# yewzijian/RegTR

Measured on AMD Instinct MI355X. Metric: point-cloud pairs/sec (3DMatch ~20k pts), higher is better.
Workload: dtype f32 (f16-pair split, 22-bit operands)

## Files before the change

### include/regtr_hip.h

```cpp
#ifndef REGTR_HIP_H
#define REGTR_HIP_H

#include <stddef.h>

#ifdef __cplusplus
extern "C" {
#endif

#define REGTR_OK 0
#define REGTR_ERR_LAUNCH (-1)
#define REGTR_ERR_ARG (-2)
#define REGTR_ERR_WORKSPACE (-3)

#define REGTR_ABI_VERSION 11
int regtr_abi_version(void);

#define REGTR_STATUS_F16_RANGE 1
#define REGTR_STATUS_NONFINITE_POSE 2


size_t regtr_grid_subsample_ws_bytes(int n_cap, int n_clouds);

int regtr_grid_subsample(const float* xyz, const int* seg_off, int n_clouds, int n_cap, float dl, float* out_xyz,
                         int* out_seg_off, void* ws, size_t ws_bytes, void* stream);

size_t regtr_grid_subsample_ordered_ws_bytes(int n_cap, int n_clouds, int row_order);
int regtr_grid_subsample_ordered(const float* xyz, const int* seg_off, int n_clouds, int n_cap, float dl, int row_order, int key_mode,
                                 int out_cap, float* out_xyz, int* out_seg_off, void* ws, size_t ws_bytes, void* stream);

size_t regtr_cellgrid_ws_bytes(int ns_cap, int n_clouds);

int regtr_cellgrid_build(const float* s_xyz, const int* s_seg_off, int n_clouds, int ns_cap, float radius, void* ws,
                         size_t ws_bytes, void* stream);

int regtr_radius_query(const float* q_xyz, const int* q_seg_off, int nq_cap, const int* s_seg_off, int ns_cap,
                       int n_clouds, float radius, int K, int order, const void* grid_ws, size_t ws_bytes, int* out_idx,
                       int* out_count, int* out_max_count, void* stream);

int regtr_radius_query_self(const int* s_seg_off, int ns_cap, int n_clouds, float radius, int K, int order, const void* grid_ws,
                            size_t ws_bytes, int* out_idx, int* out_count, int* out_max_count, void* stream);


int regtr_nearest_in_radius(const float* q_xyz, const int* q_seg_off, int nq_cap, const int* s_seg_off, int ns_cap,
                            int n_clouds, double radius, float grid_radius, const void* grid_ws, size_t ws_bytes, int* out_idx,
                            void* stream);

int regtr_overlap_avgpool(const float* ov, int ns, const int* nbr, int ld_nbr, int nq, int H, float* out, void* stream);



int regtr_rowsum_positive(const float* x, int n, int C, const float* stats, const int* seg_off, int n_seg, float slope,
                          float* flag, void* stream);

int regtr_kpconv_gather_computes_flag(int Cin, int H);

int regtr_kpconv_gather(const float* q_xyz, int nq, const float* s_xyz, int ns, const int* nbr, int H, const float* x,
                        int Cin, const float* flag, const float* s_xyzf, const float* kernel_points, int KP, float extent,
                        const float* x_stats, const int* q_seg_off, int n_seg, float slope, float* wf, int ld_wf, float* num,
                        void* stream);

int regtr_maxpool_gather(const float* x, int ns, int C, const int* nbr, int ld_nbr, int nq, int H, float* out, void* stream);

size_t regtr_instnorm_ws_bytes(int n_clouds, int max_len, int C);
int regtr_instnorm_stats(const float* x, const int* seg_off, int n_clouds, int max_len, int C, float eps, float* stats,
                         void* ws, size_t ws_bytes, void* stream);
int regtr_instnorm_apply(const float* x, const int* seg_off, int n_clouds, int max_len, int C, const float* stats,
                         const float* residual, const float* res_stats, int act, float slope, float* y, const float* row_xyz,
                         float* row_positive, void* stream);


size_t regtr_gemm_f32_ws_bytes(int M, int N, int K);
int regtr_gemm_f32(const float* A, int lda, const float* B, int ldb, float* C, int ldc, int M, int N, int K,
                   const float* bias, const float* row_div, const float* residual, int ldr, int act,
                   const float* a_stats, const int* a_seg_off, int n_seg, float a_slope, void* ws, size_t ws_bytes,
                   void* stream);

int regtr_gemm_x3_supported(int M, int N, int K);
int regtr_gemm_x3_preferred(int M, int N, int K);
size_t regtr_gemm_split_weights_bytes(int N, int K);
int regtr_gemm_split_weights(const float* W, int ld, int N, int K, int transposed, void* planes, void* stream);
int regtr_gemm_x3_f16_supported(int M, int N, int K, int with_stats);
size_t regtr_gemm_split_weights_f16_bytes(int N, int K);
int regtr_gemm_split_weights_f16(const float* W, int ld, int N, int K, int transposed, void* planes, void* stream);
size_t regtr_gemm_x3_ws_bytes(int M, int N, int K);
int regtr_gemm_x3(const float* A, int lda, const void* planes, float* C, int ldc, int M, int N, int K,
                  const float* bias, const float* row_div, const float* residual, int ldr, int act,
                  const float* a_stats, const int* a_seg_off, int n_seg, float a_slope, void* ws, size_t ws_bytes,
                  double* stat_partial, const int* stat_seg_off, int n_stat_seg, int n_planes, const void* tile_info, int* status,
                  void* stream);
int regtr_tile_segments(const int* seg_off, int n_seg, int M, int rows, void* out, void* stream);
int regtr_gemm_x3_tile_rows(int M, int N, int K);
int regtr_gemm_stream_supported(int M, int N, int K);
int regtr_gemm_stream_tile_rows(void);
int regtr_gemm_stream(const float* A, int lda, const void* planes, float* C, int ldc, int M, int N, int K,
                      const float* a_stats, float a_slope, const int* seg_off, int n_seg, const void* tile_info,
                      double* stat_partial, void* stream);
int regtr_block_tail_supported(int M, int N, int K1, int K2);
size_t regtr_block_tail_ws_bytes(int n_clouds, int max_len, int N, int K1, int K2);
int regtr_block_tail(const float* A1, int lda1, const float* a1_stats, float a1_slope, const float* row_div1, const float* A2, int lda2,
                     const float* W1, const float* W2, const int* seg_off, int n_clouds, int max_len, const void* tile_info,
                     int M, int N, int K1, int K2, float eps, float slope, float* Y, int ldy, void* ws, size_t ws_bytes,
                     float* out_stats, void* stream);

int regtr_gemm_x3_stat_tile_rows(int M, int N, int K);
int regtr_instnorm_finalize_tiles(const double* partial, const int* seg_off, int n_clouds, int C, int tile_rows, float eps,
                                  float* stats, void* stream);

int regtr_add_f32(const float* a, const float* b, size_t n, float* out, void* stream);

int regtr_layernorm(const float* x, int n, int D, const float* gamma, const float* beta, float eps, const float* add,
                    float* y, float* y_plain, void* stream);

int regtr_posemb_sine(const float* xyz, int n, int npf, int d_model, float scale, const float* dim_t, float* pe,
                      void* stream);

int regtr_posemb_mlp(const float* xyz, int n, const float* const* w_kn, const float* const* bias, int d_model, float* pe, float* acts,
                     void* stream);


int regtr_mha_fwd(const float* q, int ldq, const float* k, int ldk, const float* v, int ldv, float* out, int ldo,
                  const int* seg_off, const int* kv_of, int n_clouds, int max_len, int n_heads, int head_dim, float scale,
                  int precision, int* status, void* stream);

int regtr_cross_encoder_per_layer_params(void);
int regtr_cross_encoder_supported(int n_tok, int d_model, int d_ff, int n_heads);
size_t regtr_cross_encoder_ws_bytes(int n_tok, int d_model, int d_ff);
int regtr_cross_encoder_fwd(const float* x, int n_tok, int d_model, int d_ff, int n_heads, int n_layers,
                            const void* const* layer_params, const float* layer_eps, const float* final_gamma,
                            const float* final_beta, float final_eps, int return_intermediate, const float* pe,
                            const int* seg_off, const int* kv_self, const int* kv_cross, int n_clouds, int max_len,
                            int gemm_planes, int attn_precision, void* ws, size_t ws_bytes, float* outs, int* status, void* stream);

typedef struct {
    const float* kn;
    const void* planes;
    const void* planes16;
    int N, K;
} regtr_weight_t;
typedef struct {
    int kind;
    int strided;
    int layer;
    int n_kp;
    float extent;
    const float* kernel_points;
    regtr_weight_t unary1;
    regtr_weight_t conv;
    regtr_weight_t unary2;
    regtr_weight_t shortcut;
} regtr_encoder_block_t;
typedef struct {
    const float* points;
    int n;
    const int* conv_idx;
    const int* pool_idx;
    int K;
    int pool_width;
    const int* seg_off;
    int max_len;
} regtr_encoder_level_t;
int regtr_encoder_supported(const regtr_encoder_block_t* blocks, int n_blocks, const regtr_encoder_level_t* levels, int n_levels,
                            int n_clouds, int first, int last);
size_t regtr_encoder_ws_bytes(const regtr_encoder_block_t* blocks, int n_blocks, const regtr_encoder_level_t* levels, int n_levels,
                              int n_clouds, int first, int last, int f16_pair);
int regtr_encoder_fwd(const regtr_encoder_block_t* blocks, int n_blocks, const regtr_encoder_level_t* levels, int n_levels, int n_clouds,
                      int first, int last, const float* x_in, float* out, int f16_pair, float slope, float eps, void* ws, size_t ws_bytes,
                      int* status, void* stream);

int regtr_attn_xyz(const float* q, const float* k, const float* xyz, float* out, const int* seg_off, const int* kv_of,
                   int n_clouds, int n_total, int n_layers, int max_len, int head_dim, float scale, void* stream);

int regtr_weighted_procrustes(const float* kp, const float* corr, const float* logit, const int* seg_off, int n_pairs,
                              int n_total, int n_layers, float* pose, int* status, void* stream);

int regtr_weighted_procrustes_bwd(const float* kp, const float* corr, const float* logit, const int* seg_off, int n_pairs, int n_total,
                                  int n_layers, const float* d_pose, float* d_corr, float* d_logit, float* d_kp, float* d_weight,
                                  void* stream);


// ... 215 lines not shown
```

### regtr_amd/_lib.py

```python
import ctypes
import os
import threading

import torch

from . import context

_HERE = os.path.dirname(os.path.abspath(__file__))
LIB_PATH = os.path.join(_HERE, 'libregtr_hip.so')
if os.environ.get('REGTR_DEV', '') == '1' and os.environ.get('REGTR_VARIANT'):
    LIB_PATH = os.path.join(_HERE, f"libregtr_hip.{os.environ['REGTR_VARIANT']}.so")

_c = ctypes
_P = _c.c_void_p
_I = _c.c_int
_F = _c.c_float
_Z = _c.c_size_t
_U64 = _c.c_uint64
_U32 = _c.c_uint32
_P5 = _c.POINTER(_c.c_void_p * 5)

class Weight(_c.Structure):
    _fields_ = [('kn', _P), ('planes', _P), ('planes16', _P), ('N', _I), ('K', _I)]


class EncoderBlock(_c.Structure):
    _fields_ = [('kind', _I), ('strided', _I), ('layer', _I), ('n_kp', _I), ('extent', _F), ('kernel_points', _P),
                ('unary1', Weight), ('conv', Weight), ('unary2', Weight), ('shortcut', Weight)]


class EncoderLevel(_c.Structure):
    _fields_ = [('points', _P), ('n', _I), ('conv_idx', _P), ('pool_idx', _P), ('K', _I), ('pool_width', _I), ('seg_off', _P), ('max_len', _I)]


ABI_VERSION = 11

PARITY_SIGNATURES = {
    'regtr_parity_abi_version': (_I, []),
    'regtr_kdtree_ws_bytes': (_Z, [_I, _I]),
    'regtr_kdtree_query_scratch_bytes': (_Z, [_I]),
    'regtr_kdtree_build': (_I, [_P, _P, _I, _I, _P, _Z, _P]),
    'regtr_kdtree_radius_query': (_I, [_P, _P, _I, _P, _P, _I, _I, _F, _I, _I, _P, _Z, _P, _Z, _P, _P, _P, _P, _P]),
}

SIGNATURES = {
    'regtr_abi_version': (_I, []),
    'regtr_grid_subsample_ws_bytes': (_Z, [_I, _I]),
    'regtr_grid_subsample': (_I, [_P, _P, _I, _I, _F, _P, _P, _P, _Z, _P]),
    'regtr_grid_subsample_ordered_ws_bytes': (_Z, [_I, _I, _I]),
    'regtr_grid_subsample_ordered': (_I, [_P, _P, _I, _I, _F, _I, _I, _I, _P, _P, _P, _Z, _P]),
    'regtr_cellgrid_ws_bytes': (_Z, [_I, _I]),
    'regtr_cellgrid_build': (_I, [_P, _P, _I, _I, _F, _P, _Z, _P]),
    'regtr_radius_query': (_I, [_P, _P, _I, _P, _I, _I, _F, _I, _I, _P, _Z, _P, _P, _P, _P]),
    'regtr_radius_query_self': (_I, [_P, _I, _I, _F, _I, _I, _P, _Z, _P, _P, _P, _P]),
    'regtr_nearest_in_radius': (_I, [_P, _P, _I, _P, _I, _I, _c.c_double, _F, _P, _Z, _P, _P]),
    'regtr_overlap_avgpool': (_I, [_P, _I, _P, _I, _I, _I, _P, _P]),
    'regtr_rowsum_positive': (_I, [_P, _I, _I, _P, _P, _I, _F, _P, _P]),
    'regtr_kpconv_gather_computes_flag': (_I, [_I, _I]),
    'regtr_kpconv_gather': (_I, [_P, _I, _P, _I, _P, _I, _P, _I, _P, _P, _P, _I, _F, _P, _P, _I, _F, _P, _I, _P, _P]),
    'regtr_maxpool_gather': (_I, [_P, _I, _I, _P, _I, _I, _I, _P, _P]),
    'regtr_instnorm_ws_bytes': (_Z, [_I, _I, _I]),
    'regtr_instnorm_stats': (_I, [_P, _P, _I, _I, _I, _F, _P, _P, _Z, _P]),
    'regtr_instnorm_apply': (_I, [_P, _P, _I, _I, _I, _P, _P, _P, _I, _F, _P, _P, _P, _P]),
    'regtr_gemm_f32_ws_bytes': (_Z, [_I, _I, _I]),
    'regtr_gemm_f32': (_I, [_P, _I, _P, _I, _P, _I, _I, _I, _I, _P, _P, _P, _I, _I, _P, _P, _I, _F, _P, _Z, _P]),
    'regtr_gemm_x3_supported': (_I, [_I, _I, _I]),
    'regtr_gemm_x3_preferred': (_I, [_I, _I, _I]),
    'regtr_gemm_split_weights_bytes': (_Z, [_I, _I]),
    'regtr_gemm_split_weights': (_I, [_P, _I, _I, _I, _I, _P, _P]),
    'regtr_gemm_x3_f16_supported': (_I, [_I, _I, _I, _I]),
    'regtr_gemm_split_weights_f16_bytes': (_Z, [_I, _I]),
    'regtr_gemm_split_weights_f16': (_I, [_P, _I, _I, _I, _I, _P, _P]),
    'regtr_gemm_x3_ws_bytes': (_Z, [_I, _I, _I]),
    'regtr_gemm_x3': (_I, [_P, _I, _P, _P, _I, _I, _I, _I, _P, _P, _P, _I, _I, _P, _P, _I, _F, _P, _Z, _P, _P, _I, _I, _P, _P, _P]),
    'regtr_tile_segments': (_I, [_P, _I, _I, _I, _P, _P]),
    'regtr_gemm_x3_tile_rows': (_I, [_I, _I, _I]),
    'regtr_gemm_stream_supported': (_I, [_I, _I, _I]),
    'regtr_gemm_stream_tile_rows': (_I, []),
    'regtr_block_tail_supported': (_I, [_I, _I, _I, _I]),
    'regtr_block_tail_ws_bytes': (_Z, [_I, _I, _I, _I, _I]),
    'regtr_block_tail': (_I, [_P, _I, _P, _F, _P, _P, _I, _P, _P, _P, _I, _I, _P, _I, _I, _I, _I, _F, _F, _P, _I, _P, _Z, _P, _P]),
    'regtr_gemm_stream': (_I, [_P, _I, _P, _P, _I, _I, _I, _I, _P, _F, _P, _I, _P, _P, _P]),
    'regtr_gemm_x3_stat_tile_rows': (_I, [_I, _I, _I]),
    'regtr_instnorm_finalize_tiles': (_I, [_P, _P, _I, _I, _I, _F, _P, _P]),
    'regtr_add_f32': (_I, [_P, _P, _Z, _P, _P]),
    'regtr_layernorm': (_I, [_P, _I, _I, _P, _P, _F, _P, _P, _P, _P]),
    'regtr_posemb_sine': (_I, [_P, _I, _I, _I, _F, _P, _P, _P]),
    'regtr_posemb_mlp': (_I, [_P, _I, _P5, _P5, _I, _P, _P, _P]),
    'regtr_mha_fwd': (_I, [_P, _I, _P, _I, _P, _I, _P, _I, _P, _P, _I, _I, _I, _I, _F, _I, _P, _P]),
    'regtr_cross_encoder_per_layer_params': (_I, []),
    'regtr_cross_encoder_supported': (_I, [_I, _I, _I, _I]),
    'regtr_cross_encoder_ws_bytes': (_Z, [_I, _I, _I]),
    'regtr_cross_encoder_fwd': (_I, [_P, _I, _I, _I, _I, _I, _P, _P, _P, _P, _F, _I, _P, _P, _P, _P, _I, _I, _I, _I, _P, _Z, _P, _P, _P]),
    'regtr_encoder_supported': (_I, [_P, _I, _P, _I, _I, _I, _I]),
    'regtr_encoder_ws_bytes': (_Z, [_P, _I, _P, _I, _I, _I, _I, _I]),
    'regtr_encoder_fwd': (_I, [_P, _I, _P, _I, _I, _I, _I, _P, _P, _I, _F, _F, _P, _Z, _P, _P]),
    'regtr_attn_xyz': (_I, [_P, _P, _P, _P, _P, _P, _I, _I, _I, _I, _I, _F, _P]),
    'regtr_weighted_procrustes': (_I, [_P, _P, _P, _P, _I, _I, _I, _P, _P, _P]),
    'regtr_weighted_procrustes_bwd': (_I, [_P, _P, _P, _P, _I, _I, _I, _P, _P, _P, _P, _P, _P]),
    'regtr_infonce_ws_bytes': (_Z, [_I, _I]),
    'regtr_infonce': (_I, [_P, _I, _P, _I, _P, _P, _P, _P, _I, _I, _I, _I, _I, _F, _F, _P, _P, _P, _P, _P, _Z, _P]),
    'regtr_loss_terms': (_I, [_P, _P, _P, _P, _P, _I, _I, _P, _I, _P, _P]),
    'regtr_se3_transform': (_I, [_P, _P, _I, _I, _P, _I, _P, _P]),
    'regtr_infonce_rows': (_I, [_P, _I, _P, _I, _P, _P, _P, _P, _I, _I, _I, _I, _I, _F, _F, _P, _P, _P, _P, _P, _P, _P, _Z, _P]),
    'regtr_infonce_bwd': (_I, [_P, _I, _P, _I, _P, _P, _P, _P, _I, _I, _I, _I, _I, _I, _F, _P, _P, _P, _P, _P, _P, _F, _P, _I, _P, _I,
                               _P]),
    'regtr_circle_rows': (_I, [_P, _I, _P, _I, _P, _P, _P, _P, _I, _I, _I, _I, _I, _I, _F, _F, _F, _F, _F, _F, _F, _P, _P, _P, _P, _P, _P,
                               _P]),
    'regtr_circle_bwd': (_I, [_P, _I, _P, _I, _P, _P, _P, _P, _I, _I, _I, _I, _I, _I, _F, _F, _F, _F, _F, _F, _F, _P, _P, _P, _P, _P, _P,
                              _P, _F, _P, _I, _P, _I, _P]),
    'regtr_gemm_tn_ws_bytes': (_Z, [_I, _I, _I]),
    'regtr_gemm_tn': (_I, [_P, _I, _P, _I, _I, _I, _I, _I, _P, _I, _P, _Z, _P]),
    'regtr_corr_l1_bwd': (_I, [_P, _P, _P, _P, _I, _I, _P, _I, _P, _P, _P, _P]),
    'regtr_mha_bwd_ws_bytes': (_Z, [_I, _I]),
    'regtr_mha_bwd': (_I, [_P, _I, _P, _I, _P, _I, _P, _I, _P, _I, _P, _I, _P, _I, _P, _P, _I, _I, _I, _I, _I, _F, _P, _Z, _P]),
    'regtr_layernorm_bwd_ws_bytes': (_Z, [_I, _I]),
    'regtr_layernorm_bwd': (_I, [_P, _I, _I, _P, _F, _P, _P, _P, _P, _P, _P, _Z, _P]),
    'regtr_bias_relu_bwd_ws_bytes': (_Z, [_I, _I]),
    'regtr_bias_relu_bwd': (_I, [_P, _I, _P, _I, _P, _I, _P, _I, _I, _P, _Z, _P]),
    'regtr_nbr_transpose_ws_bytes': (_Z, [_I, _I, _I]),
    'regtr_nbr_transpose': (_I, [_P, _I, _I, _I, _P, _P, _P, _Z, _P]),
    'regtr_kpconv_gather_bwd': (_I, [_P, _P, _I, _P, _I, _I, _I, _P, _I, _F, _P, _P, _P, _P]),
    'regtr_row_div': (_I, [_P, _I, _P, _I, _I, _P, _I, _P]),
    'regtr_gemm_tn_any_ws_bytes': (_Z, [_I, _I, _I]),
    'regtr_gemm_tn_any': (_I, [_P, _I, _P, _I, _I, _I, _I, _P, _I, _P, _Z, _P]),
    'regtr_instnorm_bwd_ws_bytes': (_Z, [_I, _I, _I]),
    'regtr_instnorm_bwd': (_I, [_P, _P, _I, _I, _I, _P, _P, _P, _I, _F, _P, _P, _P, _P, _Z, _P]),
    'regtr_maxpool_argmax': (_I, [_P, _I, _I, _P, _I, _I, _I, _P, _P]),
    'regtr_maxpool_fwd_argmax': (_I, [_P, _I, _I, _P, _I, _I, _I, _P, _P, _P]),
    'regtr_maxpool_gather_bwd': (_I, [_P, _P, _I, _I, _I, _P, _P, _I, _P, _P]),
    'regtr_head_tail_bwd_ws_bytes': (_Z, [_I, _I]),
    'regtr_head_tail_bwd': (_I, [_P, _P, _P, _P, _P, _P, _I, _I, _P, _P, _P, _P, _P, _P, _P, _P, _Z, _P]),
    'regtr_bce_logits_bwd': (_I, [_P, _P, _P, _I, _P, _P]),
    'regtr_cloud_centroids': (_I, [_P, _P, _I, _I, _P, _P]),
    'regtr_augment_draws': (_I, [_P, _I, _P, _I, _U64, _U32, _I, _F, _I, _P, _P, _P, _P]),
    'regtr_shuffle_keys': (_I, [_P, _I, _I, _U64, _U32, _P, _P]),
    'regtr_augment_gather': (_I, [_P, _P, _P, _I, _P, _P, _P, _I, _I, _P, _F, _U64, _U32, _P, _P, _P]),
    'regtr_modelnet_draws': (_I, [_I, _U64, _U32, _c.c_double, _c.c_double, _P, _P, _P, _P]),
    'regtr_crop_select_lds_points': (_I, []),
    'regtr_crop_select': (_I, [_P, _P, _I, _I, _I, _P, _P, _P, _P, _I, _P, _P, _P, _P, _P, _P]),
    'regtr_modelnet_keys': (_I, [_P, _I, _I, _I, _P, _U64, _U32, _P, _P]),
    'regtr_modelnet_gather': (_I, [_P, _P, _I, _I, _P, _I, _I, _P, _P, _P, _P, _F, _F, _U64, _U32, _P, _P, _P, _P]),
    'regtr_nearest_lds_points': (_I, []),
    'regtr_nearest': (_I, [_P, _P, _I, _P, _P, _I, _I, _I, _P, _P, _P, _P, _P]),
    'regtr_segment_mean': (_I, [_P, _P, _I, _I, _P, _P]),
    'regtr_pose_metrics': (_I, [_P, _P, _I, _I, _I, _P, _P, _P]),
    'regtr_optim_norm_slice': (_I, []),
    'regtr_optim_step_slice': (_I, []),
    'regtr_optim_chunk_tensors': (_I, []),
    'regtr_grad_sumsq': (_I, [_P, _I, _P, _c.c_longlong, _P]),
    'regtr_grad_norm_finish': (_I, [_P, _c.c_longlong, _F, _P, _P]),
    'regtr_adam_step': (_I, [_P, _I, _P, _I, _P]),
    'regtr_gather_segments': (_I, [_P, _P, _P, _I, _P, _I, _I, _P, _P, _I, _I, _I, _P, _P, _P, _P]),
    'regtr_grad_pack_slice': (_I, []),
    'regtr_grad_pack': (_I, [_P, _I, _P, _c.c_longlong, _F, _I, _P]),
    'regtr_grad_pack_guarded': (_I, [_P, _I, _P, _c.c_longlong, _F, _I, _P, _P, _P]),
    'regtr_optim_guarded_chunk_tensors': (_I, []),
    'regtr_grad_norm_finish_guarded': (_I, [_P, _c.c_longlong, _F, _P, _P, _P, _P]),
    'regtr_adam_step_guarded': (_I, [_P, _I, _P, _P, _c.c_longlong, _P, _P, _P, _I, _P]),
    'regtr_adam_bias_scalars': (_I, [_c.c_double, _c.c_double, _c.c_double, _P, _I, _P, _P]),
    'regtr_icp_chunk': (_I, []),
    'regtr_icp_ws_bytes': (_Z, [_I, _I]),
    'regtr_icp_step': (_I, [_P, _P, _I, _I, _P, _I, _I, _c.c_double, _F, _P, _Z, _P, _I, _I, _c.c_double, _c.c_double, _P, _P, _P, _P, _P,
                            _P, _Z, _P]),
}
# ... 122 lines not shown
```

### regtr_amd/csrc/gemm_stream.hip

```cpp
#include "common.h"
#include "mfma_operands.h"

namespace {

constexpr int SG_WAVES = 8;
constexpr int SG_ROWS = 32 * SG_WAVES;

struct SgArgs {
    const float* A; const uint16_t* Wt; float* C;
    const float2* a_stats;
    const int* seg_off;
    const int4* tile_info;
    double2* stat_partial;
    size_t plane;
    int M, N, Kp, lda, ldc, n_seg;
    float a_slope;
};

template <int KT> __device__ __forceinline__ unsigned sg_swz(unsigned n)
{
    constexpr int CPR = 2 * KT;
    return CPR == 4 ? ((n >> 2) & 3u) : (CPR == 8 ? ((n >> 1) & 7u) : (n & 15u));
}

// ... 70 lines not shown
                }
            }
            unsigned w[4][3];
#pragma unroll
            for (int e = 0; e < 4; e++) rg_split2(row_ok ? x[2 * e] : 0.f, row_ok ? x[2 * e + 1] : 0.f, w[e]);
#pragma unroll
            for (int p = 0; p < 3; p++) fa[ks][p] = __builtin_bit_cast(bf16x8, make_uint4(w[0][p], w[1][p], w[2][p], w[3][p]));
        }
    }
    SG_STAMP();
    unsigned f_off[KT];
#pragma unroll
    for (int ks = 0; ks < KT; ks++) f_off[ks] = (unsigned)l31 * ROWB + (((unsigned)(2 * ks + hi)) ^ sg_swz<KT>((unsigned)l31)) * 16u;

    floatx16 acc[NT];
#pragma unroll
    for (int j = 0; j < NT; j++)
#pragma unroll
        for (int r = 0; r < 16; r++) acc[j][r] = 0.f;
#pragma unroll
    for (int ks = 0; ks < KT; ks++)
#pragma unroll
        for (int j = 0; j < NT; j++) {
            bf16x8 fb[3];
#pragma unroll
            for (int p = 0; p < 3; p++)
                fb[p] = __builtin_bit_cast(bf16x8, *(const uint4*)(Ws + (size_t)(p * NB + 32 * j) * ROWB + f_off[ks]));
            acc[j] = __builtin_amdgcn_mfma_f32_32x32x16_bf16(fa[ks][2], fb[0], acc[j], 0, 0, 0);
            acc[j] = __builtin_amdgcn_mfma_f32_32x32x16_bf16(fa[ks][1], fb[1], acc[j], 0, 0, 0);
            acc[j] = __builtin_amdgcn_mfma_f32_32x32x16_bf16(fa[ks][0], fb[2], acc[j], 0, 0, 0);
            acc[j] = __builtin_amdgcn_mfma_f32_32x32x16_bf16(fa[ks][1], fb[0], acc[j], 0, 0, 0);
            acc[j] = __builtin_amdgcn_mfma_f32_32x32x16_bf16(fa[ks][0], fb[1], acc[j], 0, 0, 0);
            acc[j] = __builtin_amdgcn_mfma_f32_32x32x16_bf16(fa[ks][0], fb[0], acc[j], 0, 0, 0);
        }

    const int rbase = r0 + 4 * hi;
#ifdef SG_PROF
    { float z = 0.f; for (int j = 0; j < NT; j++) z += acc[j][0]; if (z == 1.2345e30f) pt[0] = 0; }
#endif
    SG_STAMP();
    if (g.stat_partial) {
    double2* red = (double2*)(Ws + (size_t)3 * NB * ROWB);
    for (int sg = s_lo; sg <= s_hi; sg++) {
        const int c_lo = sg == s_lo ? ti.z : g.seg_off[sg], c_hi = min(sg == s_lo ? ti.w : g.seg_off[sg + 1], g.M);
#pragma unroll
        for (int j = 0; j < NT; j++) {
            double s = 0.0, q = 0.0;
#pragma unroll
            for (int r = 0; r < 16; r++) {
                const int rw = rbase + (r & 3) + 8 * (r >> 2);
                if (rw >= c_lo && rw < c_hi) { const double v = (double)acc[j][r]; s += v; q += v * v; }
            }
            s += __shfl_xor(s, 32, RG_WAVE); q += __shfl_xor(q, 32, RG_WAVE);
            if (hi == 0) red[wave * NB + 32 * j + l31] = make_double2(s, q);
        }
        __syncthreads();
        if (t < NB) {
            double2 a = red[t];
#pragma unroll
            for (int w = 1; w < SG_WAVES; w++) { const double2 b = red[w * NB + t]; a.x += b.x; a.y += b.y; }
            g.stat_partial[(size_t)(row_tile + sg) * N + n0 + t] = a;
        }
        if (sg < s_hi) __syncthreads();
    }
    }
    SG_STAMP();
#pragma unroll
    for (int j = 0; j < NT; j++)
#pragma unroll
        for (int r = 0; r < 16; r++) {
            const int rw = rbase + (r & 3) + 8 * (r >> 2);
            if (rw < g.M) g.C[(size_t)rw * g.ldc + n0 + 32 * j + l31] = acc[j][r];
        }
#ifdef SG_PROF
    SG_STAMP();
    __builtin_amdgcn_s_waitcnt(0);
    SG_STAMP();
    if (lane == 0 && (row_tile == 700 || row_tile == 1500) && n0 == 0 && (wave == 0 || wave == 5))
        printf("gemm_strip KT %d NT %d row tile %d wave %d: loads+Wcopy %lld barrier %lld split %lld mfma %lld stats %lld store-issue %lld drain %lld total %lld\n", KT, NT, row_tile, wave,
               pt[1] - pt[0], pt[2] - pt[1], pt[3] - pt[2], pt[4] - pt[3], pt[5] - pt[4], pt[6] - pt[5], pt[7] - pt[6], pt[7] - pt[0]);
#endif
}

int sg_cols_per_wg(int N, int K)
{
    for (int nb = 128; nb >= 32; nb /= 2)
        if (nb <= N && N % nb == 0 && (size_t)nb * K * 6 + (size_t)SG_WAVES * nb * 16 <= 64 * 1024) return nb;
    return 0;
}

}

extern "C" {

int regtr_gemm_stream_supported(int M, int N, int K)
{
    return (M >= 0 && (K == 32 || K == 64 || K == 128) && N >= 32 && N <= 512 && N % 32 == 0 && sg_cols_per_wg(N, K) > 0) ? 1 : 0;
}

int regtr_gemm_stream_tile_rows(void) { return SG_ROWS; }

int regtr_gemm_stream(const float* A, int lda, const void* planes, float* C, int ldc, int M, int N, int K,
                      const float* a_stats, float a_slope, const int* seg_off, int n_seg, const void* tile_info,
                      double* stat_partial, void* stream)
{
    if (!A || !planes || !C || !regtr_gemm_stream_supported(M, N, K) || lda < K || ldc < N) return RG_ERR_ARG;
    if ((lda % 4) || ((uintptr_t)A % 16) || ((uintptr_t)planes % 16)) return RG_ERR_ARG;
    if (!seg_off || n_seg < 1 || !tile_info || ((uintptr_t)tile_info % 16)) return RG_ERR_ARG;
    if (a_stats && (K > 64 || ((uintptr_t)a_stats % 16))) return RG_ERR_ARG;
    if (stat_partial && ((uintptr_t)stat_partial % 16)) return RG_ERR_ARG;
    if (M == 0) return RG_OK;
    const RgPlaneDims pd = rg_plane_dims(N, K);
    SgArgs g{A, (const uint16_t*)planes, C, (const float2*)a_stats, seg_off, (const int4*)tile_info, (double2*)stat_partial,
             pd.elems(), M, N, pd.Kp, lda, ldc, n_seg, a_slope};
    const int NB = sg_cols_per_wg(N, K);
    hipStream_t st = (hipStream_t)stream;
    const size_t lds = (size_t)3 * NB * K * 2 + (size_t)SG_WAVES * NB * 16;
    const long long n_wg = (long long)rg_cdiv(rg_cdiv(M, SG_ROWS), 8) * 8 * (N / NB);
    if (n_wg > 0x7fffffffLL) return RG_ERR_ARG;
    const dim3 grid((unsigned)n_wg);
#define SG_L3(KT_, NT_) do { if (a_stats) k_gemm_strip<KT_, NT_, (KT_ <= 4)><<<grid, SG_WAVES * RG_WAVE, lds, st>>>(g); \
                             else k_gemm_strip<KT_, NT_, false><<<grid, SG_WAVES * RG_WAVE, lds, st>>>(g); } while (0)
#define SG_L2(KT_) do { if (NB == 32) SG_L3(KT_, 1); else if (NB == 64) SG_L3(KT_, 2); else SG_L3(KT_, 4); } while (0)
    if (K == 32) SG_L2(2);
    else if (K == 64) SG_L2(4);
    else SG_L2(8);
#undef SG_L2
#undef SG_L3
    RG_RETURN_IF_LAUNCH_FAILED();
    return RG_OK;
}

}
```

### regtr_amd/ops.py

```python
import functools
import math
import operator

import torch

from . import _lib, context
from ._lib import bptr, check, dptr, iptr, ptr, raw, stream


def _ws(nbytes, device):
    return torch.empty(int(nbytes), dtype=torch.uint8, device=device)


def _ws_as(numel, dtype, device):
    return _ws(int(numel) * dtype.itemsize, device).view(dtype)


F16_OPERAND_LIMIT = 65504.0 / 2


VOXEL_KEY_MODES = {'origin': 0, 'floor': 1, 'floor_rcp': 2}


def grid_subsample(xyz, seg_off, n_cap, dl, row_order=0, key_mode=0, out_cap=None):
# ... 181 lines not shown
    ldc = out.stride(0) if M > 1 else N
    n_seg = a_seg_off.numel() - 1 if a_stats is not None else 0
    x3_ok, x3_pref, nb, x3_R, x3_rows = _x3_plan(M, N, K) if sw is not None and sw.planes is not None else (False, False, 0, 0, 0)
    ctx = context.current()
    use_f16_pair = ctx.f16_pair and not ctx.force_x3
    if ctx.force_x3:
        planes = 3
    f16_range_log = ctx.f16_range_log
    if (x3_ok and lda % 4 == 0 and a.data_ptr() % 16 == 0 and not force_f32_gemm and (N >= 64 or a_stats is None)
            and (force_x3_gemm or x3_pref)):
        ws = _ws(nb, a.device) if nb else None
        R = x3_R if want_stats is not None else 0
        partial, s_off, n_clouds = None, None, 0
        if R:
            s_off = want_stats[0]
            n_clouds = s_off.numel() - 1
            partial = _ws_as(((M + R - 1) // R + n_clouds) * N * 2, torch.float64, a.device)
        seg_rows = s_off if R else a_seg_off
        ti = None
        if seg_rows is not None and (a_seg_off is None or s_off is None or a_seg_off is s_off):
            ti = tile_segments(seg_rows, M, x3_rows)
        pl, npl = sw.planes, int(planes)
        if use_f16_pair and npl >= 2 and sw.f16_ok and f16_pair_ok(M, N, K, R > 0 or a_stats is not None or ti is not None):
            pl, npl = sw.planes16, 4
            if f16_range_log is not None:
                f16_range_log.append((M, N, K, float(a.abs().max()) if M else 0.0, float(sw.kn.abs().max())))
        tm = _GemmTimer(ctx.gemm_records, M=M, N=N, K=K, route='split GEMM (f16 pair)' if npl == 4 else f'split GEMM (bf16 x{npl})',
                        terms={4: 3, 3: 6, 2: 3, 1: 1}[npl], w_bytes={4: 4, 3: 6, 2: 4, 1: 2}[npl], fold=a_stats is not None, stats=R > 0)
        check(L.regtr_gemm_x3(raw(a), lda, bptr(pl), raw(out), ldc, M, N, K, ptr(bias), ptr(row_div),
                              raw(residual), ldr, 1 if relu else 0,
                              ptr(a_stats), iptr(a_seg_off), n_seg, a_slope, bptr(ws), nb, dptr(partial), iptr(s_off), n_clouds,
                              npl, iptr(ti), ctx.status_ptr(), stream()), 'regtr_gemm_x3')
        tm.done()
        if R:
            stats = torch.empty((n_clouds, N, 2), dtype=torch.float32, device=a.device)
            check(L.regtr_instnorm_finalize_tiles(dptr(partial), iptr(s_off), n_clouds, N, R, eps, ptr(stats), stream()),
                  'regtr_instnorm_finalize_tiles')
            return out, stats
    else:
        nb = L.regtr_gemm_f32_ws_bytes(M, N, K)
        ws = _ws(nb, a.device) if nb else None
        tm = _GemmTimer(ctx.gemm_records, M=M, N=N, K=K, route='exact-f32 MFMA', terms=0, w_bytes=4, fold=a_stats is not None, stats=False)
        check(L.regtr_gemm_f32(raw(a), lda, ptr(b_kn), N, raw(out), ldc, M, N, K, ptr(bias), ptr(row_div),
                               raw(residual), ldr, 1 if relu else 0,
                               ptr(a_stats), iptr(a_seg_off), n_seg, a_slope, bptr(ws), nb, stream()), 'regtr_gemm_f32')
        tm.done()
    if want_stats is not None:
        return out, instnorm_stats(out, want_stats[0], want_stats[1], eps)
    return out


def tile_segments(seg_off, M, rows):
    cache = getattr(seg_off, '_regtr_tiles', None)
    if cache is None:
        cache = seg_off._regtr_tiles = {}
    key = (M, rows, seg_off.data_ptr(), seg_off._version)
    t = cache.get(key)
    if t is None:
        t = torch.empty(((M + rows - 1) // rows, 4), dtype=torch.int32, device=seg_off.device)
        check(_lib.lib().regtr_tile_segments(iptr(seg_off), seg_off.numel() - 1, M, rows, iptr(t), stream()), 'regtr_tile_segments')
        for k in [k for k in cache if k[2:] != key[2:]]:
            del cache[k]
        cache[key] = t
    return t


def stream_ok(M, N, K, a, a_stats=None):
    return bool(use_stream_gemm and not force_f32_gemm and not force_x3_gemm and M >= STREAM_MIN_ROWS and a.stride(1) == 1
                and a.stride(0) % 4 == 0 and a.data_ptr() % 16 == 0 and (a_stats is None or K <= 64)
                and _lib.lib().regtr_gemm_stream_supported(M, N, K))


def gemm_stream(a, sw, seg_off, a_stats=None, a_slope=0.1, want_stats=False, eps=1e-5):
    L = _lib.lib()
    M, K = a.shape
    N = sw.N
    n_clouds = seg_off.numel() - 1
    R = L.regtr_gemm_stream_tile_rows()
    ti = tile_segments(seg_off, M, R)
    partial = None
    if want_stats:
        partial = _ws_as(((M + R - 1) // R + n_clouds) * N * 2, torch.float64, a.device)
    out = torch.empty((M, N), dtype=torch.float32, device=a.device)
    check(L.regtr_gemm_stream(raw(a), a.stride(0) if M > 1 else K, bptr(sw.planes), ptr(out), N, M, N, K, ptr(a_stats), a_slope,
                              iptr(seg_off), n_clouds, iptr(ti), dptr(partial), stream()), 'regtr_gemm_stream')
    if not want_stats:
        return out
    stats = torch.empty((n_clouds, N, 2), dtype=torch.float32, device=a.device)
    check(L.regtr_instnorm_finalize_tiles(dptr(partial), iptr(seg_off), n_clouds, N, R, eps, ptr(stats), stream()),
          'regtr_instnorm_finalize_tiles')
    return out, stats


def block_tail_ok(x1, x1_stats, f, sw1, sw2):
    M, K1 = x1.shape
    return bool(use_block_tail and not force_f32_gemm and not force_x3_gemm and M >= STREAM_MIN_ROWS and f.shape[0] == M
                and x1_stats is not None and sw1.N == sw2.N and x1.stride(1) == 1 and f.stride(1) == 1
                and x1.stride(0) % 4 == 0 and f.stride(0) % 4 == 0 and x1.data_ptr() % 16 == 0 and f.data_ptr() % 16 == 0
                and x1_stats.data_ptr() % 16 == 0 and _lib.lib().regtr_block_tail_supported(M, sw1.N, K1, f.shape[1]))


def block_tail(x1, x1_stats, f, sw1, sw2, seg_off, max_len, slope=0.1, eps=1e-5, want_stats=False):
    return _block_tail(x1, x1_stats, None, f, sw1.kn, sw2.kn, seg_off, max_len, slope, eps, want_stats)


def _block_tail(x1, x1_stats, row_div, f, w1_kn, w2_kn, seg_off, max_len, slope, eps, want_stats):
    L = _lib.lib()
    M, K1 = x1.shape
    K2, N = (f.shape[1] if f is not None else 0), w1_kn.shape[1]
    n_clouds = seg_off.numel() - 1
    nb = L.regtr_block_tail_ws_bytes(n_clouds, int(max_len), N, K1, K2)
    ws = _ws(nb, x1.device)
    ti = tile_segments(seg_off, M, 256)
    y = torch.empty((M, N), dtype=torch.float32, device=x1.device)
    st = torch.empty((2 if K2 else 1, n_clouds, N, 2), dtype=torch.float32, device=x1.device) if want_stats else None
    tm = _GemmTimer(context.current().gemm_records, M=M, N=N, K=K1 + K2, route='block tail (moments + two-source strip, bf16x3)', terms=6, w_bytes=6,
                    fold=True, stats=True, passes=2)
    check(L.regtr_block_tail(raw(x1), x1.stride(0), ptr(x1_stats), slope, ptr(row_div), raw(f) if f is not None else None,
                             f.stride(0) if f is not None else 0, ptr(w1_kn), ptr(w2_kn), iptr(seg_off), n_clouds, int(max_len),
                             iptr(ti), M, N, K1, K2, eps, slope, ptr(y), N, bptr(ws), nb, ptr(st), stream()), 'regtr_block_tail')
    tm.done()
    return (y, st) if want_stats else y


def first_block_ok(nq, Cin, KP, Cout):
    return bool(use_block_tail and not force_f32_gemm and not force_x3_gemm and Cin == 1 and KP == 15 and nq >= STREAM_MIN_ROWS
                and _lib.lib().regtr_block_tail_supported(nq, Cout, 16, 0))


def kpconv_norm_lrelu(q_xyz, s_xyz, nbr, x, w16_kn, kernel_points, extent, seg_off, max_len, xyzf=None, slope=0.1, eps=1e-5,
                      want_stats=False):
    L = _lib.lib()
    nq, H = nbr.shape
    ns = x.shape[0]
    KP = kernel_points.shape[0]
    wf = torch.empty((nq, 16), dtype=torch.float32, device=x.device)
    num = torch.empty(nq, dtype=torch.float32, device=x.device)
    rec = context.current().gather_records
    if rec is not None:
        e0, e1, e2 = (torch.cuda.Event(enable_timing=True) for _ in range(3))
        e0.record()
    check(L.regtr_kpconv_gather(ptr(q_xyz), nq, ptr(s_xyz), ns, iptr(nbr), H, ptr(x), 1, None, ptr(xyzf), ptr(kernel_points), KP,
                                float(extent), None, None, 0, slope, ptr(wf), 16, ptr(num), stream()), 'regtr_kpconv_gather')
    if rec is not None:
        e1.record()
    res = _block_tail(wf, None, num, None, w16_kn, None, seg_off, max_len, slope, eps, want_stats)
    if rec is not None:
        e2.record()
        rec.append((e0, e1, e2, nq, H, 1, w16_kn.shape[1]))
    return res


STREAM_MIN_ROWS = 131072
SMALL_REGIME_ROWS = 131072
use_stream_gemm = True
use_block_tail = True
PRENORM_MIN_ROWS = 65536
prenorm_gather = True
PREAPPLY_MIN_ROWS = 8192
assert PREAPPLY_MIN_ROWS == 8192, 'csrc/encoder.hip compiles this gate in (ENC_PREAPPLY_ROWS)'
use_one_call_cross_encoder = True
use_one_call_encoder = True
force_f32_gemm = False
force_x3_gemm = False


def layernorm(x, gamma, beta, add=None, eps=1e-5, want_plain=False, out=None):
    n, D = x.shape
    y = torch.empty_like(x) if out is None else out
    yp = torch.empty_like(x) if want_plain else None
    check(_lib.lib().regtr_layernorm(ptr(x), n, D, ptr(gamma), ptr(beta), eps, ptr(add), ptr(y), ptr(yp), stream()),
          'regtr_layernorm')
    return (y, yp) if want_plain else y


def add(a, b):
    assert a.shape == b.shape
    out = torch.empty_like(a)
    check(_lib.lib().regtr_add_f32(ptr(a), ptr(b), a.numel(), ptr(out), stream()), 'regtr_add_f32')
    return out


_posemb_tables = {}


def posemb_sine(xyz, d_model, scale=1.0, temperature=10000):
    n_dim = 3
    npf = d_model // n_dim // 2 * 2
    key = (npf, temperature, float(scale), xyz.device)
    ent = _posemb_tables.get(key)
    if ent is None:
        dim_t = torch.arange(npf, dtype=torch.float32)
        dim_t = (temperature ** (2 * torch.div(dim_t, 2, rounding_mode='trunc') / npf)).to(xyz.device)
        ent = _posemb_tables[key] = (dim_t, torch.tensor(scale * 2 * math.pi, dtype=torch.float32).item())
    dim_t, scale32 = ent
    pe = torch.empty((xyz.shape[0], d_model), dtype=torch.float32, device=xyz.device)
    check(_lib.lib().regtr_posemb_sine(ptr(xyz), xyz.shape[0], npf, d_model, scale32, ptr(dim_t), ptr(pe), stream()),
          'regtr_posemb_sine')
    return pe


POSEMB_MLP_WIDTHS = (3, 32, 64, 128, 256)
POSEMB_MLP_ACTS = 480
use_fused_posemb_mlp = True


def _posemb_mlp_check(xyz, weights):
    if not isinstance(xyz, torch.Tensor) or xyz.device.type != 'cuda':
        raise RuntimeError(f'posemb_mlp: xyz must be a GPU tensor (got {getattr(xyz, "device", type(xyz))}); there is no CPU fallback')
    if xyz.dim() != 2 or xyz.shape[1] != 3:
        raise RuntimeError(f'posemb_mlp: xyz must be (n, 3), got {tuple(xyz.shape)}')
    if len(weights) != 5:
        raise RuntimeError(f'posemb_mlp: five (weight (K, N), bias (N,)) pairs are needed, got {len(weights)}')
    d_model = int(weights[4][0].shape[1])
    widths = POSEMB_MLP_WIDTHS + (d_model,)
    for l, (w, b) in enumerate(weights):
        if tuple(w.shape) != (widths[l], widths[l + 1]) or tuple(b.shape) != (widths[l + 1],):
            raise RuntimeError(f'posemb_mlp: layer {l} must be a ({widths[l]}, {widths[l + 1]}) weight in (K, N) layout and a '
                               f'({widths[l + 1]},) bias, got {tuple(w.shape)} and {tuple(b.shape)}')
    return d_model


def posemb_mlp(xyz, weights, save=False):
    if not use_fused_posemb_mlp:
        return posemb_mlp_composed(xyz, weights, save)
    d_model = _posemb_mlp_check(xyz, weights)
    n = xyz.shape[0]
    pe = torch.empty((n, d_model), dtype=torch.float32, device=xyz.device)
    acts = torch.empty((n, POSEMB_MLP_ACTS), dtype=torch.float32, device=xyz.device) if save else None
    w5 = (_lib._c.c_void_p * 5)(*[ptr(w) for w, _ in weights])
    b5 = (_lib._c.c_void_p * 5)(*[ptr(b) for _, b in weights])
    check(_lib.lib().regtr_posemb_mlp(ptr(xyz), n, w5, b5, d_model, ptr(pe), ptr(acts), stream()), 'regtr_posemb_mlp')
    return (pe, acts) if save else pe


def posemb_mlp_composed(xyz, weights, save=False):
    d_model = _posemb_mlp_check(xyz, weights)
    n = xyz.shape[0]
    acts = torch.empty((n, POSEMB_MLP_ACTS), dtype=torch.float32, device=xyz.device) if save else None
# ... 973 lines not shown
```

Baseline: 2274.

## Add column-walking stream GEMM kernel that reuses A fragments across all N

Adds a kernel where each workgroup owns a row strip, loads and splits A once into bf16 planes, and then walks every column slot. Weight slices are double-buffered into LDS through global_load_lds DMA. The existing kernel splits columns across workgroups, so each of them reloads and resplits the same A rows; the new path removes that duplication for a fixed list of (N,K) shapes. The cost is less parallelism per launch, since there are only row-tile workgroups, plus hand-written asm waitcnt and barrier logic around the in-LDS stats reduction.

```diff
diff --git a/include/regtr_hip.h b/include/regtr_hip.h
--- a/include/regtr_hip.h
+++ b/include/regtr_hip.h
@@ -95,6 +95,10 @@
 int regtr_gemm_stream(const float* A, int lda, const void* planes, float* C, int ldc, int M, int N, int K,
                       const float* a_stats, float a_slope, const int* seg_off, int n_seg, const void* tile_info,
                       double* stat_partial, void* stream);
+int regtr_gemm_stream_form(const float* A, int lda, const void* planes, float* C, int ldc, int M, int N, int K,
+                           const float* a_stats, float a_slope, const int* seg_off, int n_seg, const void* tile_info,
+                           double* stat_partial, int form, void* stream);
+int regtr_gemm_stream_walks_columns(int N, int K, int form);
 int regtr_block_tail_supported(int M, int N, int K1, int K2);
 size_t regtr_block_tail_ws_bytes(int n_clouds, int max_len, int N, int K1, int K2);
 int regtr_block_tail(const float* A1, int lda1, const float* a1_stats, float a1_slope, const float* row_div1, const float* A2, int lda2,
diff --git a/regtr_amd/_lib.py b/regtr_amd/_lib.py
--- a/regtr_amd/_lib.py
+++ b/regtr_amd/_lib.py
@@ -81,6 +81,8 @@
     'regtr_block_tail_ws_bytes': (_Z, [_I, _I, _I, _I, _I]),
     'regtr_block_tail': (_I, [_P, _I, _P, _F, _P, _P, _I, _P, _P, _P, _I, _I, _P, _I, _I, _I, _I, _F, _F, _P, _I, _P, _Z, _P, _P]),
     'regtr_gemm_stream': (_I, [_P, _I, _P, _P, _I, _I, _I, _I, _P, _F, _P, _I, _P, _P, _P]),
+    'regtr_gemm_stream_walks_columns': (_I, [_I, _I, _I]),
+    'regtr_gemm_stream_form': (_I, [_P, _I, _P, _P, _I, _I, _I, _I, _P, _F, _P, _I, _P, _P, _I, _P]),
     'regtr_gemm_x3_stat_tile_rows': (_I, [_I, _I, _I]),
     'regtr_instnorm_finalize_tiles': (_I, [_P, _P, _I, _I, _I, _F, _P, _P]),
     'regtr_add_f32': (_I, [_P, _P, _Z, _P, _P]),
diff --git a/regtr_amd/csrc/gemm_stream.hip b/regtr_amd/csrc/gemm_stream.hip
--- a/regtr_amd/csrc/gemm_stream.hip
+++ b/regtr_amd/csrc/gemm_stream.hip
@@ -176,6 +176,206 @@
 #endif
 }
 
+constexpr int SGC_SLOT = 3 * 4096 * 2;
+constexpr int SGC_RED = SG_WAVES * 32 * 16;
+constexpr size_t SGC_LDS = 2 * SGC_SLOT + 2 * SGC_RED;
+
+typedef unsigned sgc_u4 __attribute__((ext_vector_type(4)));
+#define SGC_VM(N_) asm volatile("s_waitcnt vmcnt(%0)" :: "n"(N_) : "memory")
+#define SGC_BARRIER() asm volatile("s_waitcnt lgkmcnt(0)\n\ts_barrier" ::: "memory")
+
+__device__ __forceinline__ void sgc_dma16(const void* sbase, unsigned voff, unsigned lds_dst)
+{
+    unsigned keep;
+    asm volatile("s_mov_b32 %0, m0\n\ts_mov_b32 m0, %3\n\ts_nop 0\n\tglobal_load_lds_dwordx4 %1, %2\n\ts_mov_b32 m0, %0"
+                 : "=&s"(keep) : "v"(voff), "s"(sbase), "s"(lds_dst) : "memory");
+}
+
+__device__ __forceinline__ void sgc_store(const float* sbase, unsigned voff, float v)
+{
+    asm volatile("global_store_dword %0, %1, %2" :: "v"(voff), "v"(v), "s"(sbase) : "memory");
+}
+__device__ __forceinline__ void sgc_store16(const double2* sbase, unsigned voff, double2 v)
+{
+    asm volatile("global_store_dwordx4 %0, %1, %2\n\ts_nop 1" :: "v"(voff), "v"(__builtin_bit_cast(sgc_u4, v)), "s"(sbase) : "memory");
+}
+
+template <int KT> __device__ __forceinline__ unsigned sgc_w_off(const SgArgs& g, int wave, int lane)
+{
+    constexpr unsigned CPR = 2 * KT;
+    const unsigned rem = (unsigned)(wave * RG_WAVE + lane), n = rem / CPR, cs = rem - n * CPR;
+    return (n * (unsigned)g.Kp + ((cs ^ sg_swz<KT>(n)) * 8u)) * 2u;
+}
+template <int KT> __device__ __forceinline__ void sgc_stage(const SgArgs& g, int n0, unsigned lds_dst, unsigned w_off, int wave)
+{
+#pragma unroll
+    for (int p = 0; p < 3; p++)
+        sgc_dma16((const void*)(g.Wt + (size_t)p * g.plane + (size_t)n0 * g.Kp), w_off, lds_dst + (unsigned)(p * SG_WAVES + wave) * 1024u);
+}
+
+template <int KT, bool INFOLD>
+__global__ void __launch_bounds__(SG_WAVES* RG_WAVE, 4) k_gemm_strip_cols(SgArgs g)
+{
+    constexpr int K = 16 * KT, CPR = 2 * KT, ROWB = K * 2, SC = 4096 / K, SP = SC / 32;
+    constexpr int SGC_AFTER = 16 * SP < 63 ? 16 * SP : 63;
+    extern __shared__ __align__(16) unsigned char Ws[];
+    const int t = threadIdx.x, lane = t & 63, l31 = lane & 31, hi = lane >> 5;
+    const int wave = __builtin_amdgcn_readfirstlane(t >> 6);
+    const int row_tile = (int)blockIdx.x;
+    if (row_tile * SG_ROWS >= g.M) return;
+    const int N = g.N;
+    const int m0 = row_tile * SG_ROWS, r0 = m0 + 32 * wave;
+    const int row = r0 + l31;
+    const bool row_ok = row < g.M;
+    const bool wave_full = r0 + 32 <= g.M;
+
+    float4 raw[KT][2];
+    {
+        const float* ap = g.A + (size_t)(row_ok ? row : g.M - 1) * g.lda + 8 * hi;
+#pragma unroll
+        for (int ks = 0; ks < KT; ks++) {
+            raw[ks][0] = *(const float4*)(ap + 16 * ks);
+            raw[ks][1] = *(const float4*)(ap + 16 * ks + 4);
+        }
+    }
+    const int4 ti = g.tile_info[row_tile];
+    const unsigned lds_base = (unsigned)(unsigned long long)(rg_lds_ptr)(&Ws[0]);
+    sgc_stage<KT>(g, 0, lds_base, sgc_w_off<KT>(g, wave, lane), wave);
+    const int s_lo = ti.x, s_hi = ti.y;
+    const bool one_cloud = s_lo == s_hi;
+    bf16x8 fa[KT][3];
+    {
+        const float2* sp = nullptr;
+        if (INFOLD) {
+            const int my_seg = one_cloud ? s_lo : rg_find_segment(g.seg_off, g.n_seg, row_ok ? row : g.M - 1);
+            sp = g.a_stats + (size_t)my_seg * K + 8 * hi;
+        }
+#pragma unroll
+        for (int ks = 0; ks < KT; ks++) {
+            float x[8] = {raw[ks][0].x, raw[ks][0].y, raw[ks][0].z, raw[ks][0].w, raw[ks][1].x, raw[ks][1].y, raw[ks][1].z, raw[ks][1].w};
+            if (INFOLD) {
+#pragma unroll
+                for (int e = 0; e < 8; e += 2) {
+                    const float4 s4 = *(const float4*)(sp + 16 * ks + e);
+                    float u = (x[e] - s4.x) * s4.y;
+                    x[e] = fmaxf(u, u * g.a_slope);
+                    u = (x[e + 1] - s4.z) * s4.w;
+                    x[e + 1] = fmaxf(u, u * g.a_slope);
+                }
+            }
+            unsigned w[4][3];
+#pragma unroll
+            for (int e = 0; e < 4; e++) rg_split2(row_ok ? x[2 * e] : 0.f, row_ok ? x[2 * e + 1] : 0.f, w[e]);
+#pragma unroll
+            for (int p = 0; p < 3; p++) fa[ks][p] = __builtin_bit_cast(bf16x8, make_uint4(w[0][p], w[1][p], w[2][p], w[3][p]));
+            if constexpr (KT == 8) __builtin_amdgcn_sched_barrier(0);
+        }
+    }
+    SGC_VM(0);
+    __syncthreads();
+
+    const int nslot = (N + SC - 1) / SC;
+    int par = 0;
+    for (int s = 0; s < nslot; s++) {
+#define SGC_LANE() unsigned tl = (unsigned)t; asm volatile("" : "+v"(tl)); const int lane = (int)(tl & 63u), l31 = lane & 31, hi = lane >> 5
+        const bool more = s + 1 < nslot;
+        if (more) { SGC_LANE(); (void)l31; (void)hi; sgc_stage<KT>(g, (s + 1) * SC, lds_base + (unsigned)((s + 1) & 1) * SGC_SLOT, sgc_w_off<KT>(g, wave, lane), wave); }
+        const int npass = min(SP, (N - s * SC) >> 5);
+#pragma unroll 1
+        for (int j = 0; j < npass; j++) {
+            const int n0 = s * SC + 32 * j;
+            floatx16 acc;
+#pragma unroll
+            for (int r = 0; r < 16; r++) acc[r] = 0.f;
+            {
+            SGC_LANE();
+            const unsigned f_base = (unsigned)l31 * ROWB;
+            const unsigned f_swz = (unsigned)hi ^ sg_swz<KT>((unsigned)l31);
+#pragma unroll
+            for (int ks = 0; ks < KT; ks++) {
+                unsigned fo = (unsigned)(s & 1) * SGC_SLOT + (unsigned)(32 * j) * ROWB + f_base + (((unsigned)(2 * ks)) ^ f_swz) * 16u;
+                const unsigned char* fp = Ws + fo;
+                if constexpr (KT == 8) {
+                    bf16x8 b0 = __builtin_bit_cast(bf16x8, *(const uint4*)fp);
+                    bf16x8 bx = __builtin_bit_cast(bf16x8, *(const uint4*)(fp + (size_t)SC * ROWB));
+                    acc = __builtin_amdgcn_mfma_f32_32x32x16_bf16(fa[ks][2], b0, acc, 0, 0, 0);
+                    acc = __builtin_amdgcn_mfma_f32_32x32x16_bf16(fa[ks][1], bx, acc, 0, 0, 0);
+                    __builtin_amdgcn_sched_barrier(0);
+                    asm volatile("" : "+v"(fo));
+                    const unsigned char* fq = Ws + fo;
+                    bx = __builtin_bit_cast(bf16x8, *(const uint4*)(fq + (size_t)2 * SC * ROWB));
+                    acc = __builtin_amdgcn_mfma_f32_32x32x16_bf16(fa[ks][0], bx, acc, 0, 0, 0);
+                    acc = __builtin_amdgcn_mfma_f32_32x32x16_bf16(fa[ks][1], b0, acc, 0, 0, 0);
+                    __builtin_amdgcn_sched_barrier(0);
+                    bx = __builtin_bit_cast(bf16x8, *(const uint4*)(fq + (size_t)SC * ROWB));
+                    acc = __builtin_amdgcn_mfma_f32_32x32x16_bf16(fa[ks][0], bx, acc, 0, 0, 0);
+                    acc = __builtin_amdgcn_mfma_f32_32x32x16_bf16(fa[ks][0], b0, acc, 0, 0, 0);
+                    __builtin_amdgcn_sched_barrier(0);
+                } else {
+                    bf16x8 fb[3];
+#pragma unroll
+                    for (int p = 0; p < 3; p++) fb[p] = __builtin_bit_cast(bf16x8, *(const uint4*)(fp + (size_t)p * SC * ROWB));
+                    acc = __builtin_amdgcn_mfma_f32_32x32x16_bf16(fa[ks][2], fb[0], acc, 0, 0, 0);
+                    acc = __builtin_amdgcn_mfma_f32_32x32x16_bf16(fa[ks][1], fb[1], acc, 0, 0, 0);
+                    acc = __builtin_amdgcn_mfma_f32_32x32x16_bf16(fa[ks][0], fb[2], acc, 0, 0, 0);
+                    acc = __builtin_amdgcn_mfma_f32_32x32x16_bf16(fa[ks][1], fb[0], acc, 0, 0, 0);
+                    acc = __builtin_amdgcn_mfma_f32_32x32x16_bf16(fa[ks][0], fb[1], acc, 0, 0, 0);
+                    acc = __builtin_amdgcn_mfma_f32_32x32x16_bf16(fa[ks][0], fb[0], acc, 0, 0, 0);
+                }
+            }
+            }
+            asm volatile("s_nop 7\n\ts_nop 3" : "+v"(acc));
+            {
+                SGC_LANE();
+                const int rbase = r0 + 4 * hi;
+                const unsigned c_off = ((unsigned)(4 * hi) * (unsigned)g.ldc + (unsigned)l31) * 4u;
+                const float* cw = g.C + (size_t)r0 * g.ldc + n0;
+                if (wave_full) {
+#pragma unroll
+                    for (int r = 0; r < 16; r++) sgc_store(cw + (size_t)((r & 3) + 8 * (r >> 2)) * g.ldc, c_off, acc[r]);
+                } else {
+#pragma unroll
+                    for (int r = 0; r < 16; r++)
+                        if (rbase + (r & 3) + 8 * (r >> 2) < g.M) sgc_store(cw + (size_t)((r & 3) + 8 * (r >> 2)) * g.ldc, c_off, acc[r]);
+                }
+            }
+            const bool hand = more && j == npass - 1;
+            if (hand) { if (wave_full) SGC_VM(SGC_AFTER); else SGC_VM(0); }
+            if (g.stat_partial) {
+                int c_lo = ti.z, c_hi = min(ti.w, g.M);
+#pragma unroll 1
+                for (int sg = s_lo;;) {
+                    double2* red = (double2*)(Ws + 2 * SGC_SLOT + (size_t)par * SGC_RED);
+                    SGC_LANE();
+                    const int rbase = r0 + 4 * hi;
+                    asm volatile("" : "+v"(acc));
+                    const unsigned d0 = (unsigned)(rbase - c_lo), span = (unsigned)(c_hi - c_lo);
+                    double sm = 0.0, q = 0.0;
+#pragma unroll
+                    for (int r = 0; r < 16; r++) {
+                        const double v = (double)(d0 + (unsigned)((r & 3) + 8 * (r >> 2)) < span ? acc[r] : 0.f);
+                        sm += v; q += v * v;
+                        if constexpr (KT == 8) __builtin_amdgcn_sched_barrier(0);
+                    }
+                    sm += __shfl_xor(sm, 32, RG_WAVE); q += __shfl_xor(q, 32, RG_WAVE);
+                    if (hi == 0) red[wave * 32 + l31] = make_double2(sm, q);
+                    SGC_BARRIER();
+                    if (tl < 32u) {
+                        double2 a = red[tl];
+#pragma unroll
+                        for (int w = 1; w < SG_WAVES; w++) { const double2 b = red[w * 32 + tl]; a.x += b.x; a.y += b.y; }
+                        sgc_store16(g.stat_partial + (size_t)(row_tile + sg) * N + n0, tl * 16u, a);
+                    }
+                    par ^= 1;
+                    if (++sg > s_hi) break;
+                    c_lo = __builtin_amdgcn_readfirstlane(g.seg_off[sg]); c_hi = min(__builtin_amdgcn_readfirstlane(g.seg_off[sg + 1]), g.M);
+                }
+            } else if (hand) SGC_BARRIER();
+        }
+    }
+#undef SGC_LANE
+}
+
 int sg_cols_per_wg(int N, int K)
 {
     for (int nb = 128; nb >= 32; nb /= 2)
@@ -183,6 +383,12 @@
     return 0;
 }
 
+bool sg_walks_columns(int N, int K)
+{
+    return (K == 128 && (N == 96 || N == 128 || N == 256 || N == 512)) || (K == 64 && (N == 192 || N == 256 || N == 512)) ||
+           (K == 32 && (N == 192 || N == 256));
+}
+
 }
 
 extern "C" {
@@ -194,11 +400,11 @@
 
 int regtr_gemm_stream_tile_rows(void) { return SG_ROWS; }
 
-int regtr_gemm_stream(const float* A, int lda, const void* planes, float* C, int ldc, int M, int N, int K,
-                      const float* a_stats, float a_slope, const int* seg_off, int n_seg, const void* tile_info,
-                      double* stat_partial, void* stream)
-{
-    if (!A || !planes || !C || !regtr_gemm_stream_supported(M, N, K) || lda < K || ldc < N) return RG_ERR_ARG;
+int regtr_gemm_stream_form(const float* A, int lda, const void* planes, float* C, int ldc, int M, int N, int K,
+                           const float* a_stats, float a_slope, const int* seg_off, int n_seg, const void* tile_info,
+                           double* stat_partial, int form, void* stream)
+{
+    if (!A || !planes || !C || !regtr_gemm_stream_supported(M, N, K) || lda < K || ldc < N || form < 0 || form > 2) return RG_ERR_ARG;
     if ((lda % 4) || ((uintptr_t)A % 16) || ((uintptr_t)planes % 16)) return RG_ERR_ARG;
     if (!seg_off || n_seg < 1 || !tile_info || ((uintptr_t)tile_info % 16)) return RG_ERR_ARG;
     if (a_stats && (K > 64 || ((uintptr_t)a_stats % 16))) return RG_ERR_ARG;
@@ -209,8 +415,20 @@
              pd.elems(), M, N, pd.Kp, lda, ldc, n_seg, a_slope};
     const int NB = sg_cols_per_wg(N, K);
     hipStream_t st = (hipStream_t)stream;
+    const int row_wg = rg_cdiv(rg_cdiv(M, SG_ROWS), 8) * 8;
+    if (regtr_gemm_stream_walks_columns(N, K, form)) {
+        const dim3 grid((unsigned)row_wg);
+#define SGC_L(KT_) do { if (a_stats) k_gemm_strip_cols<KT_, (KT_ <= 4)><<<grid, SG_WAVES * RG_WAVE, SGC_LDS, st>>>(g); \
+                        else k_gemm_strip_cols<KT_, false><<<grid, SG_WAVES * RG_WAVE, SGC_LDS, st>>>(g); } while (0)
+        if (K == 32) SGC_L(2);
+        else if (K == 64) SGC_L(4);
+        else SGC_L(8);
+#undef SGC_L
+        RG_RETURN_IF_LAUNCH_FAILED();
+        return RG_OK;
+    }
     const size_t lds = (size_t)3 * NB * K * 2 + (size_t)SG_WAVES * NB * 16;
-    const long long n_wg = (long long)rg_cdiv(rg_cdiv(M, SG_ROWS), 8) * 8 * (N / NB);
+    const long long n_wg = (long long)row_wg * (N / NB);
     if (n_wg > 0x7fffffffLL) return RG_ERR_ARG;
     const dim3 grid((unsigned)n_wg);
 #define SG_L3(KT_, NT_) do { if (a_stats) k_gemm_strip<KT_, NT_, (KT_ <= 4)><<<grid, SG_WAVES * RG_WAVE, lds, st>>>(g); \
@@ -225,4 +443,17 @@
     return RG_OK;
 }
 
-}
+int regtr_gemm_stream_walks_columns(int N, int K, int form)
+{
+    const int NB = sg_cols_per_wg(N, K);
+    return (NB > 0 && N / NB >= 2 && (form == 2 || (form == 0 && sg_walks_columns(N, K)))) ? 1 : 0;
+}
+
+int regtr_gemm_stream(const float* A, int lda, const void* planes, float* C, int ldc, int M, int N, int K,
+                      const float* a_stats, float a_slope, const int* seg_off, int n_seg, const void* tile_info,
+                      double* stat_partial, void* stream)
+{
+    return regtr_gemm_stream_form(A, lda, planes, C, ldc, M, N, K, a_stats, a_slope, seg_off, n_seg, tile_info, stat_partial, 0, stream);
+}
+
+}
diff --git a/regtr_amd/ops.py b/regtr_amd/ops.py
--- a/regtr_amd/ops.py
+++ b/regtr_amd/ops.py
@@ -287,8 +287,9 @@
     if want_stats:
         partial = _ws_as(((M + R - 1) // R + n_clouds) * N * 2, torch.float64, a.device)
     out = torch.empty((M, N), dtype=torch.float32, device=a.device)
-    check(L.regtr_gemm_stream(raw(a), a.stride(0) if M > 1 else K, bptr(sw.planes), ptr(out), N, M, N, K, ptr(a_stats), a_slope,
-                              iptr(seg_off), n_clouds, iptr(ti), dptr(partial), stream()), 'regtr_gemm_stream')
+    form = 0 if strip_columns is None else (2 if strip_columns else 1)
+    check(L.regtr_gemm_stream_form(raw(a), a.stride(0) if M > 1 else K, bptr(sw.planes), ptr(out), N, M, N, K, ptr(a_stats), a_slope,
+                                   iptr(seg_off), n_clouds, iptr(ti), dptr(partial), form, stream()), 'regtr_gemm_stream_form')
     if not want_stats:
         return out
     stats = torch.empty((n_clouds, N, 2), dtype=torch.float32, device=a.device)
@@ -360,6 +361,7 @@
 SMALL_REGIME_ROWS = 131072
 use_stream_gemm = True
 use_block_tail = True
+strip_columns = None
 PRENORM_MIN_ROWS = 65536
 prenorm_gather = True
 PREAPPLY_MIN_ROWS = 8192
```

New measurement: 2314, median of 6. 1.02x the previous value.
